# HaileyMai/Self-supervised-scene-generation-with-semantic-segmentation

Measured on NVIDIA B200. Metric: raycast fwd+bwd rays/s, higher is better.
Workload: dtype f32

## Files before the change

include/spsg_raycast.h:

```cpp
#ifndef SPSG_RAYCAST_H_
#define SPSG_RAYCAST_H_

#include <stddef.h>
#include <stdint.h>

#ifdef __cplusplus
extern "C" {
#endif

#if defined(__GNUC__)
#define SPSG_API __attribute__((visibility("default")))
#else
#define SPSG_API
#endif

#define SPSG_SEMANTIC_CHANNELS 14
#define SPSG_GRAD_CHANNELS 21

enum {
    SPSG_OK = 0,
    SPSG_ERR_INVALID_ARGUMENT = 1,
    SPSG_ERR_CUDA = 2,
    SPSG_ERR_WORKSPACE_TOO_SMALL = 3
};

enum {
    SPSG_FLAG_NO_CLIP = 1u << 0,
    SPSG_FLAG_NO_BRICK_SKIP = 1u << 1,
    SPSG_FLAG_RECORD_HITS = 1u << 2,
    SPSG_FLAG_GRADS_CLEARED = 1u << 3,
    SPSG_FLAG_SMEM_MAPS = 1u << 5,
    SPSG_FLAG_GLOBAL_MAPS = 1u << 6,
    SPSG_FLAG_PACKED_LOCS = 1u << 8,
    SPSG_FLAG_INDEX_PREBUILT = 1u << 7,
    SPSG_FLAG_DETERMINISTIC_GRADS = 1u << 4,
    SPSG_FLAG_VIEW_NORMALS = 1u << 9
};

typedef struct spsg_raycast_params {
    int32_t width, height;
    float depth_min, depth_max, thresh_sample_dist, ray_increment;
    int32_t dimx, dimy, dimz;
    int32_t num_chunks;
    int32_t views_per_chunk;
    int32_t max_pixels_per_voxel;
    int64_t num_locs;
    uint32_t flags;
    uint32_t reserved;
} spsg_raycast_params;

typedef struct spsg_loss_targets {
    const float *target_depth;
    const float *target_color;
    const float *weight_color;
    const uint8_t *target_label;
    const float *class_weight;
    float voxelsize;
    float weight_depth, weight_color_loss, weight_semantic;
} spsg_loss_targets;

typedef struct spsg_grad_buffers {
    float *d_color;
    float *d_depth;
    float *d_normal;
    float *d_semantic;
} spsg_grad_buffers;

#define SPSG_LOSS_OUT_FLOATS 8

SPSG_API const char *spsg_version(void);
SPSG_API const char *spsg_last_error(void);

SPSG_API void spsg_timing_enable(int on);
SPSG_API int spsg_timing_read(int which, double *total_ms, int *launches);

SPSG_API size_t spsg_workspace_bytes(const spsg_raycast_params *p);

SPSG_API int spsg_build_index(const int64_t *locs, int64_t num_locs, int32_t *sparse_mapping, int32_t num_chunks,
                              int32_t dimz, int32_t dimy, int32_t dimx, void *stream);

SPSG_API int spsg_raycast_forward(const spsg_raycast_params *p, const int32_t *sparse_mapping, const int64_t *locs,
                                  const float *vals_sdf, const float *vals_color, const float *vals_normal,
                                  const float *vals_semantic, const float *view_matrix, const float *intrinsics,
                                  float *image_color, float *image_depth, float *image_normal,
                                  float *image_semantic, int32_t *mapping3dto2d, int32_t *mapping3dto2d_num,
                                  void *workspace, size_t workspace_bytes, void *stream);

SPSG_API int spsg_raycast_forward_indexed(const spsg_raycast_params *p, int32_t *sparse_mapping, const int64_t *locs,
// ... 148 lines not shown
```

self-supervised-scene-generation-with-semantic-segmentation_b200/_native.py:

```python
import ctypes
import os

_HERE = os.path.dirname(os.path.abspath(__file__))
LIB_PATH = os.environ.get("SPSG_RAYCAST_LIB", os.path.join(_HERE, "lib", "libspsg_raycast.so"))

SPSG_FLAG_NO_CLIP = 1 << 0
SPSG_FLAG_NO_BRICK_SKIP = 1 << 1
SPSG_FLAG_RECORD_HITS = 1 << 2
SPSG_FLAG_GRADS_CLEARED = 1 << 3
SPSG_FLAG_DETERMINISTIC_GRADS = 1 << 4
SPSG_FLAG_SMEM_MAPS = 1 << 5
SPSG_FLAG_GLOBAL_MAPS = 1 << 6
SPSG_FLAG_INDEX_PREBUILT = 1 << 7
SPSG_FLAG_PACKED_LOCS = 1 << 8
SPSG_FLAG_VIEW_NORMALS = 1 << 9
SPSG_LOSS_OUT_FLOATS = 8
SPSG_DTYPE_F32 = 0
SPSG_DTYPE_BF16 = 1
SPSG_DEPTH_MAX_FILL_ROUNDS = 64

EXPORTS = (
    "spsg_version", "spsg_last_error", "spsg_workspace_bytes", "spsg_build_index", "spsg_raycast_forward",
    "spsg_raycast_forward_indexed", "spsg_raycast_backward", "spsg_raycast_occ", "spsg_raycast_forward_loss",
    "spsg_raycast_backward_loss", "spsg_raycast_backward_loss_upstream", "spsg_timing_enable", "spsg_timing_read",
    "spsg_normals_forward", "spsg_normals_backward", "spsg_normals_forward_views", "spsg_normals_backward_views",
    "spsg_losses2d_forward", "spsg_losses2d_backward",
    "spsg_depth_bilateral_filter", "spsg_depth_median_fill", "spsg_depth_to_cameraspace", "spsg_depth_to_normals",
    "spsg_depth_compute_normals",
    "spsg_sparsify_scratch_bytes", "spsg_sparsify_count", "spsg_sparsify_locs", "spsg_sparsify_locs_indexed",
    "spsg_dense_gather", "spsg_dense_scatter",
    "spsg_sparsify_count_bf16", "spsg_sparsify_locs_bf16", "spsg_sparsify_locs_indexed_bf16",
    "spsg_dense_gather_strided", "spsg_dense_scatter_strided",
    "spsg_labels_from_render", "spsg_pack_locs_host",
)


class Params(ctypes.Structure):
    _fields_ = [
        ("width", ctypes.c_int32), ("height", ctypes.c_int32),
        ("depth_min", ctypes.c_float), ("depth_max", ctypes.c_float),
        ("thresh_sample_dist", ctypes.c_float), ("ray_increment", ctypes.c_float),
        ("dimx", ctypes.c_int32), ("dimy", ctypes.c_int32), ("dimz", ctypes.c_int32),
        ("num_chunks", ctypes.c_int32), ("views_per_chunk", ctypes.c_int32),
        ("max_pixels_per_voxel", ctypes.c_int32),
        ("num_locs", ctypes.c_int64),
        ("flags", ctypes.c_uint32), ("reserved", ctypes.c_uint32),
    ]


class LossTargets(ctypes.Structure):
    _fields_ = [
        ("target_depth", ctypes.c_void_p), ("target_color", ctypes.c_void_p), ("weight_color", ctypes.c_void_p),
        ("target_label", ctypes.c_void_p), ("class_weight", ctypes.c_void_p),
        ("voxelsize", ctypes.c_float), ("weight_depth", ctypes.c_float), ("weight_color_loss", ctypes.c_float),
        ("weight_semantic", ctypes.c_float),
    ]


class DensePayload(ctypes.Structure):
    _fields_ = [("dense", ctypes.c_void_p), ("sparse", ctypes.c_void_p), ("channels", ctypes.c_int32),
                ("reserved", ctypes.c_int32)]


class DenseHead(ctypes.Structure):
    _fields_ = [("dense", ctypes.c_void_p), ("sparse", ctypes.c_void_p), ("strides", ctypes.c_int64 * 5),
                ("extent", ctypes.c_int64), ("channels", ctypes.c_int32), ("dtype", ctypes.c_int32)]


# ... 148 lines not shown
```

self-supervised-scene-generation-with-semantic-segmentation_b200/csrc/spsg_common.cuh:

```cuda
#pragma once

constexpr int kFineLog2 = 2;
constexpr int kFine = 1 << kFineLog2;
constexpr int kSuper = 8;
constexpr float kBoxEps = 1.0f / 64.0f;
constexpr float kFracGuard = 1.0f / 256.0f;
constexpr int kMaxFastDim = 8192;
constexpr int kLossSlots = 64;

enum { kKindSurface = 0, kKindEmpty = 1, kKindPos = 2, kKindNeg = 3 };

thread_local char g_err[512] = "";

int fail(int code, const char *msg) {
    snprintf(g_err, sizeof(g_err), "%s", msg);
    return code;
}
int fail_cuda(cudaError_t e, const char *where) {
    snprintf(g_err, sizeof(g_err), "%s: %s", where, cudaGetErrorString(e));
    return SPSG_ERR_CUDA;
}
#define CUDA_TRY(x)                                      \
    do {                                                 \
        cudaError_t e_ = (x);                            \
        if (e_ != cudaSuccess) return fail_cuda(e_, #x); \
    } while (0)

inline size_t align_up(size_t v, size_t a) { return (v + a - 1) / a * a; }

struct EventPair { cudaEvent_t a, b; };
bool g_timing = false;
std::vector<EventPair> g_ev[2];
std::mutex g_timing_mu;

struct ScopedKernelTimer {
    int which; cudaStream_t st; EventPair ev; bool on;
    ScopedKernelTimer(int w, cudaStream_t s) : which(w), st(s), on(g_timing) {
        if (on) {
            on = cudaEventCreate(&ev.a) == cudaSuccess && cudaEventCreate(&ev.b) == cudaSuccess;
            if (on) cudaEventRecord(ev.a, st);
        }
    }
    ~ScopedKernelTimer() {
        if (on) {
            cudaEventRecord(ev.b, st);
            std::lock_guard<std::mutex> lk(g_timing_mu);
            g_ev[which].push_back(ev);
        }
    }
};

struct Layout {
    int nbx, nby, nbz;
    size_t bpc;
    size_t dense_off, dense_bytes;
    int wpr;
    size_t vpc;
    size_t vbit_off, vbit_bytes;
    size_t bmap_off, bmap_bytes;
    size_t marks_off, marks_bytes;
    size_t zero_off, zero_bytes;
    size_t head_off;
    size_t tiles_off, tiles_bytes;
    size_t arrive_off, arrive_bytes;
    size_t loss_off, loss_bytes;
    size_t list_off, list_bytes;
    size_t hits_off, hits_bytes;
    size_t total;
};

Layout make_layout(const spsg_raycast_params *p) {
    Layout L;
    L.nbx = (p->dimx + kFine - 1) >> kFineLog2;
    L.nby = (p->dimy + kFine - 1) >> kFineLog2;
    L.nbz = (p->dimz + kFine - 1) >> kFineLog2;
    L.bpc = align_up((size_t)L.nbx * L.nby * L.nbz, 16);
    const int F = p->views_per_chunk > 0 ? p->views_per_chunk : 1;
    const size_t cells = (size_t)p->num_chunks * p->dimz * p->dimy * p->dimx;
    size_t off = 0;
    L.dense_off = off;
    L.dense_bytes = align_up(cells * sizeof(float), 256);
    off += L.dense_bytes;
    L.wpr = (p->dimx + 31) / 32;
    L.vpc = align_up((size_t)p->dimz * p->dimy * L.wpr, 2);
    L.vbit_off = off;
    L.vbit_bytes = align_up((size_t)p->num_chunks * L.vpc * sizeof(uint2), 256);
    off += L.vbit_bytes;
    L.bmap_off = off;
    L.bmap_bytes = align_up((size_t)p->num_chunks * L.bpc, 256);
    off += L.bmap_bytes;
    L.marks_off = off;
    L.marks_bytes = align_up((size_t)p->num_chunks * L.bpc, 256);
    off += L.marks_bytes;
    L.zero_off = off;
    L.head_off = off;
    off += 256;
    L.tiles_off = off;
    L.tiles_bytes = align_up((size_t)p->num_chunks * sizeof(int32_t), 256);
    off += L.tiles_bytes;
    L.arrive_off = off;
    L.arrive_bytes = align_up((size_t)p->num_chunks * ((L.nbz + 7) / 8) * ((L.nby + 7) / 8) * L.wpr * sizeof(int32_t), 256);
    off += L.arrive_bytes;
    L.loss_off = off;
    L.loss_bytes = align_up((size_t)kLossSlots * 8 * sizeof(double), 256);
    off += L.loss_bytes;
    L.zero_bytes = off - L.zero_off;
    L.list_off = off;
    L.list_bytes = align_up((size_t)(p->num_locs > 0 ? p->num_locs : 0) * F * 2 * sizeof(int32_t), 256);
    off += L.list_bytes;
    L.hits_off = off;
    L.hits_bytes = align_up((size_t)p->num_chunks * F * p->width * p->height * sizeof(int32_t), 256);
    off += L.hits_bytes;
    L.total = off;
    return L;
}
```

self-supervised-scene-generation-with-semantic-segmentation_b200/csrc/spsg_forward.cuh:

```cuda
#pragma once


#ifdef SPSG_STATS
__device__ unsigned long long g_stats[48];
__device__ int g_tile_stats[131072][8];
#define STAT_MAX(k, v) atomicMax(&g_stats[k], (unsigned long long)(v))
#define STAT_ADD(k, v) atomicAdd(&g_stats[k], (unsigned long long)(v))
#if SPSG_STATS == 1
#define EVT_ADD(k, v) STAT_ADD(k, v)
#else
#define EVT_ADD(k, v)
#endif
#else
#define STAT_ADD(k, v)
#define STAT_MAX(k, v)
#define EVT_ADD(k, v)
#endif

struct LossArgs {
    const float *target_depth, *target_color, *weight_color;
    const uint8_t *target_label;
    const float *class_weight;
    float voxelsize;
    double *accum;
    float *loss_out;
    int32_t *done;
    float w_depth, w_color, w_sem;
};

__device__ __forceinline__ void finalize_loss_warp(const double *acc, float *__restrict__ out, float w_depth, float w_color,
                                                   float w_sem, bool has_depth, bool has_color, bool has_sem, int lane);

struct ForwardArgs {
    const int32_t *sparse_mapping;
    const float *vals_sdf, *vals_color, *vals_normal, *vals_semantic;
    const float *view_matrix, *intrinsics;
    float *image_color, *image_depth, *image_normal, *image_semantic;
    int32_t *mapping3dto2d, *mapping3dto2d_num;
    const float *dense;
    const uint2 *vbits;
    const uint8_t *bmap;
    size_t vpc, bpc;
    int wpr;
    int maps_in_smem;
    int32_t *tile_counter;
    int32_t *list_count;
    int2 *list;
    int32_t *hits;
    int width, height;
    float depth_min, depth_max, thresh, inc;
    int dimx, dimy, dimz;
    int vx, vy, vz;
    int nbx, nby, nbz;
    int num_chunks, views, max_pixels;
    long long num_locs;
    unsigned flags;
    int vec_ok;
    float guard;
    LossArgs loss;
    spsg_grad_buffers clear;
    long long clear_rows;
};

constexpr int kTileW = 16, kTileH = 8;
constexpr int kTilePix = kTileW * kTileH;

constexpr int kWarpW = 8, kWarpH = 4;
constexpr int kFwdWarps = 24;
#ifndef SPSG_FWD_WARPS_LARGE
#define SPSG_FWD_WARPS_LARGE 28
#endif
constexpr int kFwdWarpsLarge = SPSG_FWD_WARPS_LARGE;
constexpr int kFwdThreads = kFwdWarps * 32;
constexpr int kStageFloats = 14 * 32;
__host__ __device__ constexpr size_t fwd_smem_fixed(int warps) { return 128 + (size_t)warps * kStageFloats * sizeof(float); }
constexpr size_t kFwdSmemFixed = fwd_smem_fixed(kFwdWarpsLarge);
constexpr size_t kFwdSmemMax = 232448 - 1024;

__device__ __forceinline__ float warp_sum(float v) {
#pragma unroll
    for (int o = 16; o > 0; o >>= 1) v += __shfl_xor_sync(0xffffffffu, v, o);
    return v;
}

__device__ __forceinline__ uint32_t smem_u32(const void *p) { return (uint32_t)__cvta_generic_to_shared(p); }
__device__ __forceinline__ void mbar_init(uint64_t *bar, unsigned count) {
    asm volatile("mbarrier.init.shared::cta.b64 [%0], %1;" ::"r"(smem_u32(bar)), "r"(count) : "memory");
    asm volatile("fence.mbarrier_init.release.cluster;" ::: "memory");
}
__device__ __forceinline__ void mbar_expect_tx(uint64_t *bar, unsigned bytes) {
    asm volatile("mbarrier.arrive.expect_tx.shared::cta.b64 _, [%0], %1;" ::"r"(smem_u32(bar)), "r"(bytes) : "memory");
}
__device__ __forceinline__ void bulk_copy_g2s(void *dst, const void *src, unsigned bytes, uint64_t *bar) {
    asm volatile("cp.async.bulk.shared::cluster.global.mbarrier::complete_tx::bytes [%0], [%1], %2, [%3];" ::"r"(
                     smem_u32(dst)),
                 "l"(src), "r"(bytes), "r"(smem_u32(bar))
                 : "memory");
}
// ... 178 lines not shown
            int img, view, wx0, wy0;
#ifdef SPSG_STATS
            long long clk0;
#endif
        };
        auto prepare = [&](int tile, TileRay &q) {
            const int view = tile / tiles_per_image, tt = tile - view * tiles_per_image;
            const int blk = tt >> 2, sub = tt & 3;
            const int by = blk / blocks_x, bx = blk - by * blocks_x;
            const int wx0 = (bx * 2 + (sub & 1)) * kWarpW, wy0 = (by * 2 + (sub >> 1)) * kWarpH;
            const int img = chunk * a.views + view;
            q.view = view; q.img = img; q.wx0 = wx0; q.wy0 = wy0;
            q.inside = wx0 < a.width && wy0 < a.height;
            if (q.inside) {
                const unsigned ux = wx0 + (lane & 7), uy = wy0 + (lane >> 3);
                const bool active = ux < (unsigned)a.width && uy < (unsigned)a.height;
                const unsigned pix = uy * a.width + ux;
                const size_t gpix = (size_t)img * a.width * a.height + pix;

#ifdef SPSG_STATS
                q.clk0 = clock64();
#endif
                const Ray r = setup_ray(a.view_matrix + (size_t)img * 16, a.intrinsics + (size_t)img * 4,
                                        active ? ux : 0u, active ? uy : 0u, a.depth_min, a.depth_max);
                const float invx = r.dx != 0.0f ? rcp_approx(r.dx) : 0.0f, invy = r.dy != 0.0f ? rcp_approx(r.dy) : 0.0f,
                            invz = r.dz != 0.0f ? rcp_approx(r.dz) : 0.0f;
                const float kx = r.dx != 0.0f ? ((r.dx > 0.0f ? -kBoxEps : kBoxEps) - r.camx) * invx : kInf;
                const float ky = r.dy != 0.0f ? ((r.dy > 0.0f ? -kBoxEps : kBoxEps) - r.camy) * invy : kInf;
                const float kz = r.dz != 0.0f ? ((r.dz > 0.0f ? -kBoxEps : kBoxEps) - r.camz) * invz : kInf;
                const int sxm = r.dx > 0.0f ? -1 : 0, sym = r.dy > 0.0f ? -1 : 0, szm = r.dz > 0.0f ? -1 : 0;
                float ray = r.t0, t_end = active ? r.t1 : -kInf;
                int jump_cap = 1 << 22;
                {
                    const float top = fmaxf(fabsf(r.t1), 1.0f);
                    const float ulp = __uint_as_float(__float_as_uint(top) & 0x7f800000u) * 1.1920928955078125e-07f;
                    const float cap = (0.5f * kBoxEps) / ulp;
                    jump_cap = cap < 4194304.0f ? max(1, __float2int_rd(cap)) : (1 << 22);
                }
                if (clip && active) {
                    float tin = -kInf, tout = kInf;
#define SPSG_SLAB(o, d, inv, lo, hi)                                        \
    if ((d) != 0.0f) {                                                      \
        const float ta_ = ((lo) - (o)) * (inv), tb_ = ((hi) - (o)) * (inv); \
        tin = fmaxf(tin, fminf(ta_, tb_));                                  \
        tout = fminf(tout, fmaxf(ta_, tb_));                                \
    } else if ((o) < (lo) || (o) > (hi)) {                                  \
        tin = kInf;                                                         \
        tout = -kInf;                                                       \
    }
                    SPSG_SLAB(r.camx, r.dx, invx, -kBoxEps, (float)(a.dimx - 1) + kBoxEps)
                    SPSG_SLAB(r.camy, r.dy, invy, -kBoxEps, (float)(a.dimy - 1) + kBoxEps)
                    SPSG_SLAB(r.camz, r.dz, invz, -kBoxEps, (float)(a.dimz - 1) + kBoxEps)
#undef SPSG_SLAB
                    const float margin = 0.0625f;
                    if (!(tin <= tout)) {
                        t_end = -kInf;
                    } else {
                        t_end = fminf(t_end, tout + margin);
                        while (ray < tin - margin - a.inc && ray < t_end) {
                            const int want = max(1, min(__float2int_rd((tin - margin - ray) * inv_inc) - 1, jump_cap));
                            ray = step_advance(s_steps, a.inc, ray, want);
                        }
                        for (int k = 0; k < 6 && ray < t_end; k++) {
                            const int ix = __float2int_rd(__fmaf_rn(r.dx, ray, r.camx)), iy = __float2int_rd(__fmaf_rn(r.dy, ray, r.camy)),
                                      iz = __float2int_rd(__fmaf_rn(r.dz, ray, r.camz));
                            if ((unsigned)ix < (unsigned)a.vx && (unsigned)iy < (unsigned)a.vy && (unsigned)iz < (unsigned)a.vz) break;
                            if (!skip_ok) break;
                            ray = __fadd_rn(ray, a.inc);
                        }
                    }
                }
                q.r = r; q.invx = invx; q.invy = invy; q.invz = invz; q.kx = kx; q.ky = ky; q.kz = kz;
                q.sxm = sxm; q.sym = sym; q.szm = szm; q.ray = ray; q.t_end = t_end; q.jump_cap = jump_cap;
                q.pix = pix; q.gpix = gpix; q.active = active;
            }
        };
        TileRay q;
        q.inside = false;
        if (tile < tile_limit) prepare(bind_chunk(tile), q);
        if (kSmemMaps) mbar_wait(mbar, phase);

        while (tile < tile_limit) {
            int next = tile_limit;
            if (lane == 0 && static_tiles < tile_limit) next = static_tiles + atomicAdd(counter, 1);
            if (q.inside) {
                const Ray r = q.r;
                const float invx = q.invx, invy = q.invy, invz = q.invz, kx = q.kx, ky = q.ky, kz = q.kz;
                const int sxm = q.sxm, sym = q.sym, szm = q.szm, jump_cap = q.jump_cap;
                float ray = q.ray;
                const float t_end = q.t_end;
                const unsigned pix = q.pix;
                const size_t gpix = q.gpix;
                const bool active = q.active;
                const int img = q.img, view = q.view, wx0 = q.wx0, wy0 = q.wy0;
                int hit = -1;
                float depth = 0.0f;
#ifdef SPSG_STATS
                const long long clk0 = q.clk0;
                long long clk_march = 0, clk_refine = 0;
                int my_iters = 0;
                const long long clk1 = clock64(), clk1b = clk1;
#endif

                float last_sdf = 0.0f, last_alpha = 0.0f;
                bool last_lazy = false;
                float dist = 0.0f;
// ... 327 lines not shown
```

self-supervised-scene-generation-with-semantic-segmentation_b200/csrc/spsg_prep.cuh:

```cuda
#pragma once


constexpr int kFillRegions = 3;
struct FillArgs {
    uint32_t *ptr[kFillRegions];
    size_t words[kFillRegions];
    uint32_t value[kFillRegions];
};

__global__ void __launch_bounds__(256) fill_kernel(const FillArgs a) {
    const size_t tid = (size_t)blockIdx.x * blockDim.x + threadIdx.x, stride = (size_t)gridDim.x * blockDim.x;
#pragma unroll
    for (int r = 0; r < kFillRegions; r++) {
        uint32_t *p = a.ptr[r];
        const size_t n = a.words[r];
        if (!p || n == 0) continue;
        const uint32_t v = a.value[r];
        if ((reinterpret_cast<uintptr_t>(p) & 15u) == 0) {
            const size_t n4 = n >> 2;
            uint4 *p4 = reinterpret_cast<uint4 *>(p);
            for (size_t i = tid; i < n4; i += stride) p4[i] = make_uint4(v, v, v, v);
            for (size_t i = (n4 << 2) + tid; i < n; i += stride) p[i] = v;
        } else {
            for (size_t i = tid; i < n; i += stride) p[i] = v;
        }
    }
}

__global__ void __launch_bounds__(256) index_packed_kernel(const uint32_t *__restrict__ cells, long long n,
                                                           int32_t *__restrict__ sparse_mapping,
                                                           const float *__restrict__ vals_sdf, float *__restrict__ dense,
                                                           int32_t *__restrict__ num, int views, unsigned long long grid_cells) {
    const long long i = (long long)blockIdx.x * blockDim.x + threadIdx.x;
    if (i >= n) return;
    if (num)
        for (int f = 0; f < views; f++) num[(long long)f * n + i] = 0;
    const unsigned cell = __ldg(cells + i);
    if ((unsigned long long)cell >= grid_cells) return;
    sparse_mapping[cell] = (int32_t)i;
    if (dense) dense[cell] = __ldg(vals_sdf + i);
}

template <bool kWriteIndex>
__global__ void __launch_bounds__(256) index_kernel(const longlong4 *__restrict__ locs, long long n,
                                                    int32_t *__restrict__ sparse_mapping,
                                                    const float *__restrict__ vals_sdf, float *__restrict__ dense,
                                                    int32_t *__restrict__ num, int views, int dimz, int dimy,
                                                    int dimx, int num_chunks) {
    const long long i = (long long)blockIdx.x * blockDim.x + threadIdx.x;
    if (i >= n) return;
    if (num)
        for (int f = 0; f < views; f++) num[(long long)f * n + i] = 0;
    const longlong4 l = locs[i];
    const long long z = l.x, y = l.y, x = l.z, b = l.w;
    if ((unsigned long long)z >= (unsigned long long)dimz || (unsigned long long)y >= (unsigned long long)dimy ||
        (unsigned long long)x >= (unsigned long long)dimx || b < 0 || b >= num_chunks)
        return;
    const long long cell = ((b * dimz + z) * dimy + y) * dimx + x;
    if (kWriteIndex) sparse_mapping[cell] = (int32_t)i;
    if (dense) dense[cell] = __ldg(vals_sdf + i);
}

__host__ __device__ constexpr uint8_t block_map_byte(int r1, int r2, int r3, int r4) {
    const int r[5] = {0, r1, r2, r3, r4};
    int lu = 0, le = 0;
    for (int l = 1; l <= 4; l++) {
        if (!(r[l] & 4) && (r[l] & 3) != 3) lu = l;
        if (r[l] == 0) le = l;
    }
    if (lu == 0) return 0;
    const int kind = (le == lu) ? kKindEmpty : (r[lu] & 1) ? kKindPos : kKindNeg;
    return (uint8_t)((kind << 3) | lu);
}

struct BlockLut { uint8_t v[4096]; };
constexpr BlockLut make_block_lut() {
    BlockLut t{};
    for (int i = 0; i < 4096; i++) t.v[i] = block_map_byte(i & 7, (i >> 3) & 7, (i >> 6) & 7, (i >> 9) & 7);
    return t;
}
__device__ const BlockLut kBlockLut = make_block_lut();

constexpr float kTiny = 1e-30f, kHuge = 3e38f;

__global__ void __launch_bounds__(128) cell_class_kernel(const float *__restrict__ dense, uint2 *__restrict__ vbits,
                                                         size_t vpc, uint8_t *__restrict__ marks,
                                                         int dimz, int dimy, int dimx, int wpr, int nby, int nbx,
                                                         size_t bpc, uint8_t *__restrict__ bmap, int32_t *__restrict__ arrive,
                                                         int nbz) {
    const unsigned kFull = 0xffffffffu;
    const int lane = threadIdx.x & 31;
    const int w = blockIdx.x * 4 + (threadIdx.x >> 5);
    if (w >= nby * wpr) return;
    const int yb = w / wpr, xw = w - yb * wpr;
    const int zb = blockIdx.y, chunk = blockIdx.z;
    const int y0 = yb * kFine, z0 = zb * kFine;
    const unsigned plane = (unsigned)dimy * (unsigned)dimx;
    const unsigned x = (unsigned)(xw * 32 + lane);
    const bool in_x = x < (unsigned)dimx, in_x1 = x + 1u < (unsigned)dimx;
    const unsigned o00 = ((unsigned)chunk * (unsigned)dimz + (unsigned)z0) * plane + (unsigned)y0 * (unsigned)dimx + x;
    unsigned pres[5][5], posm[5][5], negm[5][5];
#pragma unroll
    for (int dz = 0; dz < 5; dz++)
#pragma unroll
        for (int dy = 0; dy < 5; dy++) {
            const bool row = y0 + dy < dimy && z0 + dz < dimz;
            const float *__restrict__ q = dense + (o00 + (unsigned)dz * plane + (unsigned)dy * (unsigned)dimx);
            const float a = (row && in_x) ? __ldg(q) : CUDART_NAN_F;
            const float n = (row && in_x1) ? __ldg(q + 1) : CUDART_NAN_F;
            pres[dz][dy] = __ballot_sync(kFull, a == a && n == n);
            posm[dz][dy] = __ballot_sync(kFull, a > kTiny && a < kHuge && n > kTiny && n < kHuge);
            negm[dz][dy] = __ballot_sync(kFull, a < -kTiny && a > -kHuge && n < -kTiny && n > -kHuge);
        }
    unsigned any_pos = 0u, any_neg = 0u, any_mix = 0u;
    const unsigned v00 = (unsigned)chunk * (unsigned)vpc + ((unsigned)z0 * (unsigned)dimy + (unsigned)y0) * (unsigned)wpr + (unsigned)xw;
#pragma unroll
    for (int dz = 0; dz < 4; dz++)
#pragma unroll
        for (int dy = 0; dy < 4; dy++) {
            const int y = y0 + dy, z = z0 + dz;
            const unsigned v = pres[dz][dy] & pres[dz][dy + 1] & pres[dz + 1][dy] & pres[dz + 1][dy + 1];
            const unsigned vp = posm[dz][dy] & posm[dz][dy + 1] & posm[dz + 1][dy] & posm[dz + 1][dy + 1];
            const unsigned vn = negm[dz][dy] & negm[dz][dy + 1] & negm[dz + 1][dy] & negm[dz + 1][dy + 1];
            any_pos |= vp; any_neg |= vn; any_mix |= v & ~vp & ~vn;
            if (lane == 0 && y < dimy && z < dimz)
                vbits[v00 + ((unsigned)dz * (unsigned)dimy + (unsigned)dy) * (unsigned)wpr] = make_uint2(v & ~vn, v & ~vp);
        }
    if (lane < 8) {
        const int bx = xw * 8 + lane;
        if (bx < nbx)
            marks[(size_t)chunk * bpc + ((size_t)zb * nby + yb) * nbx + bx] =
                (uint8_t)((((any_pos >> (4 * lane)) & 0xfu) ? 1 : 0) | (((any_neg >> (4 * lane)) & 0xfu) ? 2 : 0) |
                          (((any_mix >> (4 * lane)) & 0xfu) ? 4 : 0));
    }
    const int sby = (nby + 7) >> 3, sbz = (nbz + 7) >> 3;
    const int sy = yb >> 3, sz = zb >> 3;
    const int rows_y = min(8, nby - sy * 8), rows_z = min(8, nbz - sz * 8);
    __threadfence();
    int prev = 0;
    if (lane == 0) prev = atomicAdd(arrive + ((size_t)chunk * sbz + sz) * sby * wpr + (size_t)sy * wpr + xw, 1);
    prev = __shfl_sync(kFull, prev, 0);
    if (prev != rows_y * rows_z - 1) return;
    __threadfence();
    const int zl = lane >> 2, yl = (lane & 3) * 2;
    uint32_t rb[2][2] = {{0u, 0u}, {0u, 0u}};
    const int nx = min(8, nbx - xw * 8);
#pragma unroll
    for (int r = 0; r < 2; r++) {
        const int gy = sy * 8 + yl + r, gz = sz * 8 + zl;
        if (gy < nby && gz < nbz) {
            const uint8_t *src = marks + (size_t)chunk * bpc + ((size_t)gz * nby + gy) * nbx + xw * 8;
            if ((nbx & 7) == 0) {
                const uint2 v2 = __ldcg(reinterpret_cast<const uint2 *>(src));
                rb[r][0] = v2.x; rb[r][1] = v2.y;
            } else {
                for (int k = 0; k < nx; k++) rb[r][k >> 2] |= (uint32_t)__ldcg(src + k) << (8 * (k & 3));
            }
        }
    }
    auto xpair = [](uint32_t v) { const uint32_t t = v | ((v >> 8) & 0x00ff00ffu); return (t & 0x00ff00ffu) | ((t & 0x00ff00ffu) << 8); };
    uint32_t r8[2];
#pragma unroll
    for (int h = 0; h < 2; h++) {
        uint32_t v = xpair(rb[0][h] | rb[1][h]);
        v |= __shfl_xor_sync(kFull, v, 4);
        r8[h] = v;
    }
    uint32_t r16[2];
#pragma unroll
    for (int h = 0; h < 2; h++) {
        uint32_t v = r8[h];
        v |= v >> 16; v |= v >> 8; v &= 0xffu;
        v |= __shfl_xor_sync(kFull, v, 1);
        v |= __shfl_xor_sync(kFull, v, 8);
        r16[h] = v;
    }
    uint32_t r32 = r16[0] | r16[1];
    r32 |= __shfl_xor_sync(kFull, r32, 2);
    r32 |= __shfl_xor_sync(kFull, r32, 16);
    const uint8_t *__restrict__ lut = kBlockLut.v;
#pragma unroll
    for (int r = 0; r < 2; r++) {
        const int gy = sy * 8 + yl + r, gz = sz * 8 + zl;
        if (gy < nby && gz < nbz) {
            uint8_t *dst = bmap + (size_t)chunk * bpc + ((size_t)gz * nby + gy) * nbx + xw * 8;
            uint32_t out[2] = {0u, 0u};
// ... 15 lines not shown
```

self-supervised-scene-generation-with-semantic-segmentation_b200/csrc/spsg_raycast.cu:

```cuda
#include <cuda_runtime.h>
#include <math_constants.h>
#include <stdint.h>
#include <stdio.h>
#include <string.h>

#include <algorithm>
#include <mutex>
#include <vector>

#include "spsg_raycast.h"

namespace {

#include "spsg_common.cuh"
#include "spsg_fp32.cuh"
#include "spsg_prep.cuh"
#include "spsg_forward.cuh"
#include "spsg_backward.cuh"
#include "spsg_losses2d.cuh"
#include "spsg_occ.cuh"
#include "spsg_normals.cuh"


int check_params(const spsg_raycast_params *p) {
// ... 23 lines not shown
        cudaDeviceGetAttribute(&sms, cudaDevAttrMultiProcessorCount, dev);
        cached[dev] = sms > 0 ? sms : 148;
    }
    return cached[dev];
}

LossArgs make_loss_args(const spsg_loss_targets *t, double *accum) {
    LossArgs L;
    memset(&L, 0, sizeof(L));
    if (t) {
        L.target_depth = t->target_depth; L.target_color = t->target_color; L.weight_color = t->weight_color;
        L.target_label = t->target_label; L.class_weight = t->class_weight; L.voxelsize = t->voxelsize;
    }
    L.accum = accum;
    L.loss_out = nullptr; L.done = nullptr;
    if (t) { L.w_depth = t->weight_depth; L.w_color = t->weight_color_loss; L.w_sem = t->weight_semantic; }
    return L;
}

int launch_forward(const spsg_raycast_params *p, bool build_index, int32_t *sparse_mapping, const int64_t *locs,
                   const float *vals_sdf, const float *vals_color, const float *vals_normal,
                   const float *vals_semantic, const float *view_matrix, const float *intrinsics, float *image_color,
                   float *image_depth, float *image_normal, float *image_semantic, int32_t *mapping3dto2d,
                   int32_t *mapping3dto2d_num, const spsg_loss_targets *targets, float *loss_out,
                   const spsg_grad_buffers *clear_grads, void *workspace, size_t workspace_bytes, cudaStream_t st) {
    if (int rc = check_params(p)) return rc;
    if (p->max_pixels_per_voxel <= 0) return fail(SPSG_ERR_INVALID_ARGUMENT, "max_pixels_per_voxel must be positive");
    if (!sparse_mapping || !view_matrix || !intrinsics || !image_color || !image_depth || !image_normal ||
        !image_semantic || !mapping3dto2d || !mapping3dto2d_num)
        return fail(SPSG_ERR_INVALID_ARGUMENT, "NULL tensor pointer");
    if (p->num_locs > 0 && (!locs || !vals_sdf || !vals_color || !vals_normal || !vals_semantic))
        return fail(SPSG_ERR_INVALID_ARGUMENT, "NULL voxel tensor pointer");
    if (!aligned16(view_matrix) || !aligned16(intrinsics))
        return fail(SPSG_ERR_INVALID_ARGUMENT, "view_matrix / intrinsics must be 16-byte aligned");
    const bool packed = (p->flags & SPSG_FLAG_PACKED_LOCS) != 0;
    if (p->num_locs > 0 && ((reinterpret_cast<uintptr_t>(vals_semantic) & 7u) || (reinterpret_cast<uintptr_t>(locs) & (packed ? 3u : 15u))))
        return fail(SPSG_ERR_INVALID_ARGUMENT, "vals_semantic must be 8-byte and locs 16-byte (packed: 4-byte) aligned");
    if (packed && !build_index) return fail(SPSG_ERR_INVALID_ARGUMENT, "packed locs need an entry point that builds the index");
    if (packed && (unsigned long long)p->num_chunks * p->dimz * p->dimy * p->dimx >= 0xffffffffull)
        return fail(SPSG_ERR_INVALID_ARGUMENT, "packed locs need fewer than 2^32 - 1 cells");
    if (reinterpret_cast<uintptr_t>(sparse_mapping) & 3u) return fail(SPSG_ERR_INVALID_ARGUMENT, "sparse_mapping must be 4-byte aligned");
    if (targets && !loss_out) return fail(SPSG_ERR_INVALID_ARGUMENT, "loss_out is NULL");
    const Layout L = make_layout(p);
    if (!workspace || workspace_bytes < L.total) return fail(SPSG_ERR_WORKSPACE_TOO_SMALL, "workspace too small");
    if (reinterpret_cast<uintptr_t>(workspace) & 255u) return fail(SPSG_ERR_INVALID_ARGUMENT, "workspace must be 256-byte aligned");
    uint8_t *ws = (uint8_t *)workspace;
    float *dense = (float *)(ws + L.dense_off);
    uint2 *vbits = (uint2 *)(ws + L.vbit_off);
    uint8_t *bmap = ws + L.bmap_off, *marks = ws + L.marks_off;
    double *accum = (double *)(ws + L.loss_off);
    const size_t cells = (size_t)p->num_chunks * p->dimz * p->dimy * p->dimx;
    const int sms = sm_count();
    const bool prebuilt = (p->flags & SPSG_FLAG_INDEX_PREBUILT) && p->num_locs > 0;

    {
        FillArgs f;
        memset(&f, 0, sizeof(f));
        f.ptr[0] = build_index ? (uint32_t *)sparse_mapping : nullptr; f.words[0] = cells; f.value[0] = 0xffffffffu;
        f.ptr[1] = (uint32_t *)dense; f.words[1] = L.dense_bytes / 4; f.value[1] = 0xffffffffu;
        if (prebuilt) {
            f.ptr[0] = (uint32_t *)mapping3dto2d_num; f.words[0] = (size_t)p->views_per_chunk * p->num_locs; f.value[0] = 0u;
            f.ptr[1] = nullptr; f.words[1] = 0;
        }
        f.ptr[2] = (uint32_t *)(ws + L.zero_off); f.words[2] = L.zero_bytes / 4; f.value[2] = 0u;
        if (clear_grads && p->num_locs > 0 &&
            (!clear_grads->d_color || !clear_grads->d_depth || !clear_grads->d_normal || !clear_grads->d_semantic))
            return fail(SPSG_ERR_INVALID_ARGUMENT, "NULL gradient pointer in clear_grads");
        const size_t vecs = ((prebuilt ? f.words[0] : cells * (build_index ? 2 : 1)) + L.zero_bytes / 4) / 4;
        const unsigned blocks = (unsigned)std::min<size_t>((vecs + 1023) / 1024 + 1, (size_t)sms * 8);
        fill_kernel<<<blocks, 256, 0, st>>>(f);
        CUDA_TRY(cudaGetLastError());
    }
    if (p->num_locs > 0 && !prebuilt) {
        const unsigned blocks = (unsigned)((p->num_locs + 255) / 256);
        if (packed)
            index_packed_kernel<<<blocks, 256, 0, st>>>((const uint32_t *)locs, p->num_locs, sparse_mapping, vals_sdf, dense,
                                                        mapping3dto2d_num, p->views_per_chunk, (unsigned long long)cells);
        else if (build_index)
            index_kernel<true><<<blocks, 256, 0, st>>>((const longlong4 *)locs, p->num_locs, sparse_mapping, vals_sdf,
                                                       dense, mapping3dto2d_num, p->views_per_chunk, p->dimz, p->dimy,
                                                       p->dimx, p->num_chunks);
        else
            index_kernel<false><<<blocks, 256, 0, st>>>((const longlong4 *)locs, p->num_locs, sparse_mapping, vals_sdf,
                                                        dense, mapping3dto2d_num, p->views_per_chunk, p->dimz, p->dimy,
                                                        p->dimx, p->num_chunks);
        CUDA_TRY(cudaGetLastError());
    }
    ForwardArgs a;
    memset(&a, 0, sizeof(a));
    const size_t map_bytes = L.vpc * sizeof(uint2) + L.bpc;
    a.maps_in_smem = kFwdSmemFixed + map_bytes <= kFwdSmemMax && !(p->flags & SPSG_FLAG_GLOBAL_MAPS) &&
                     (p->num_chunks == 1 || (p->flags & SPSG_FLAG_SMEM_MAPS));
    {
        const dim3 cgrid((unsigned)((L.nby * L.wpr + 3) / 4), (unsigned)L.nbz, (unsigned)p->num_chunks);
        cell_class_kernel<<<cgrid, 128, 0, st>>>(dense, vbits, L.vpc, marks, p->dimz, p->dimy, p->dimx, L.wpr, L.nby, L.nbx, L.bpc,
                                                 bmap, (int32_t *)(ws + L.arrive_off), L.nbz);
        CUDA_TRY(cudaGetLastError());
    }
    a.sparse_mapping = sparse_mapping;
    a.vals_sdf = vals_sdf; a.vals_color = vals_color; a.vals_normal = vals_normal; a.vals_semantic = vals_semantic;
    a.view_matrix = view_matrix; a.intrinsics = intrinsics;
    a.image_color = image_color; a.image_depth = image_depth; a.image_normal = image_normal;
    a.image_semantic = image_semantic;
    a.mapping3dto2d = mapping3dto2d; a.mapping3dto2d_num = mapping3dto2d_num;
    a.dense = dense; a.vbits = vbits; a.bmap = bmap; a.vpc = L.vpc; a.bpc = L.bpc; a.wpr = L.wpr;
    a.tile_counter = (int32_t *)(ws + L.tiles_off);
    a.num_chunks = p->num_chunks;
    a.list_count = (int32_t *)(ws + L.head_off);
    a.list = (int2 *)(ws + L.list_off);
    a.hits = (p->flags & SPSG_FLAG_RECORD_HITS) ? (int32_t *)(ws + L.hits_off) : nullptr;
    a.width = p->width; a.height = p->height;
    a.depth_min = p->depth_min; a.depth_max = p->depth_max; a.thresh = p->thresh_sample_dist; a.inc = p->ray_increment;
    a.dimx = p->dimx; a.dimy = p->dimy; a.dimz = p->dimz;
    {
        const bool maps = !(p->flags & SPSG_FLAG_NO_BRICK_SKIP) && std::max(p->dimx, std::max(p->dimy, p->dimz)) <= kMaxFastDim;
        a.vx = maps ? p->dimx - 1 : 0; a.vy = maps ? p->dimy - 1 : 0; a.vz = maps ? p->dimz - 1 : 0;
    }
    a.nbx = L.nbx; a.nby = L.nby; a.nbz = L.nbz;
    a.views = p->views_per_chunk; a.max_pixels = p->max_pixels_per_voxel;
    a.num_locs = p->num_locs;
    a.flags = p->flags;
    a.vec_ok = (p->width % 4 == 0) && aligned16(image_color) && aligned16(image_depth) && aligned16(image_normal) &&
               aligned16(image_semantic);
    {
        int k = 0;
        while ((1 << k) < std::max(p->dimx, std::max(p->dimy, p->dimz))) k++;
        a.guard = std::min(kFracGuard, std::max(ldexpf(1.0f, k - 21), ldexpf(1.0f, -18)));
    }
    a.loss = make_loss_args(targets, accum);
    a.loss.loss_out = loss_out;
    a.loss.done = (int32_t *)(ws + L.head_off) + 16;
    if (clear_grads && p->num_locs > 0) {
        a.clear = *clear_grads;
        a.clear_rows = p->num_locs;
    }
    const long long tiles_x = (p->width + kWarpW - 1) / kWarpW, tiles_y = (p->height + kWarpH - 1) / kWarpH;
    const long long all_tiles = ((tiles_x + 1) / 2) * ((tiles_y + 1) / 2) * 4 * p->views_per_chunk * p->num_chunks;
    const unsigned grid = (unsigned)std::max<long long>(1, std::min<long long>(sms, all_tiles));
    const bool large = all_tiles >= (long long)sms * 4 * kFwdWarpsLarge;
    const bool view_normals = (p->flags & SPSG_FLAG_VIEW_NORMALS) && p->views_per_chunk > 1;
    const int warps = large ? kFwdWarpsLarge : kFwdWarps;
    const size_t dyn = fwd_smem_fixed(warps) + (a.maps_in_smem ? map_bytes : 0);
    {
        static std::mutex mu;
        static bool configured[64] = {false};
        int dev = 0;
        CUDA_TRY(cudaGetDevice(&dev));
        std::lock_guard<std::mutex> lk(mu);
        if (dev < 0 || dev >= 64 || !configured[dev]) {
#define SPSG_SET_SMEM(L, M, W, VN) CUDA_TRY(cudaFuncSetAttribute(raycast_forward_kernel<L, M, W, VN>, cudaFuncAttributeMaxDynamicSharedMemorySize, (int)kFwdSmemMax))
#define SPSG_SET_SMEM_ALL(VN)                                                                                   \
    SPSG_SET_SMEM(true, true, kFwdWarps, VN); SPSG_SET_SMEM(false, true, kFwdWarps, VN);                         \
    SPSG_SET_SMEM(true, false, kFwdWarps, VN); SPSG_SET_SMEM(false, false, kFwdWarps, VN);                       \
    SPSG_SET_SMEM(true, true, kFwdWarpsLarge, VN); SPSG_SET_SMEM(false, true, kFwdWarpsLarge, VN);               \
    SPSG_SET_SMEM(true, false, kFwdWarpsLarge, VN); SPSG_SET_SMEM(false, false, kFwdWarpsLarge, VN)
            SPSG_SET_SMEM_ALL(false);
            SPSG_SET_SMEM_ALL(true);
#undef SPSG_SET_SMEM_ALL
#undef SPSG_SET_SMEM
// ... 446 lines not shown
```

Baseline: 4.888 billion.

## Splat occupied voxel bricks into per-tile depth bounds to tighten ray intervals

Adds a per-image, per-screen-tile near/far depth bound. The fill kernel computes camera matrices, and the cell classification kernel projects each non-empty brick's box onto screen tiles, recording min-near and max-far with atomics. The forward raycast intersects its box-slab interval with these tile bounds, so rays skip empty space before and after the occupied geometry and tiles with no geometry stop early. The cost is extra work, atomics and workspace during prep, and the bounds must be conservative or results change.

```diff
diff --git a/include/spsg_raycast.h b/include/spsg_raycast.h
--- a/include/spsg_raycast.h
+++ b/include/spsg_raycast.h
@@ -34,6 +34,7 @@
     SPSG_FLAG_PACKED_LOCS = 1u << 8,
     SPSG_FLAG_INDEX_PREBUILT = 1u << 7,
     SPSG_FLAG_DETERMINISTIC_GRADS = 1u << 4,
+    SPSG_FLAG_NO_TILE_BOUNDS = 1u << 10,
     SPSG_FLAG_VIEW_NORMALS = 1u << 9
 };
 
diff --git a/self-supervised-scene-generation-with-semantic-segmentation_b200/_native.py b/self-supervised-scene-generation-with-semantic-segmentation_b200/_native.py
--- a/self-supervised-scene-generation-with-semantic-segmentation_b200/_native.py
+++ b/self-supervised-scene-generation-with-semantic-segmentation_b200/_native.py
@@ -14,6 +14,7 @@
 SPSG_FLAG_INDEX_PREBUILT = 1 << 7
 SPSG_FLAG_PACKED_LOCS = 1 << 8
 SPSG_FLAG_VIEW_NORMALS = 1 << 9
+SPSG_FLAG_NO_TILE_BOUNDS = 1 << 10
 SPSG_LOSS_OUT_FLOATS = 8
 SPSG_DTYPE_F32 = 0
 SPSG_DTYPE_BF16 = 1
diff --git a/self-supervised-scene-generation-with-semantic-segmentation_b200/csrc/spsg_common.cuh b/self-supervised-scene-generation-with-semantic-segmentation_b200/csrc/spsg_common.cuh
--- a/self-supervised-scene-generation-with-semantic-segmentation_b200/csrc/spsg_common.cuh
+++ b/self-supervised-scene-generation-with-semantic-segmentation_b200/csrc/spsg_common.cuh
@@ -59,7 +59,10 @@
     size_t vbit_off, vbit_bytes;
     size_t bmap_off, bmap_bytes;
     size_t marks_off, marks_bytes;
+    size_t cams_off, cams_bytes;
+    int quads_x, quads;
     size_t zero_off, zero_bytes;
+    size_t bounds_off, bounds_bytes;
     size_t head_off;
     size_t tiles_off, tiles_bytes;
     size_t arrive_off, arrive_bytes;
@@ -92,6 +95,12 @@
     L.marks_off = off;
     L.marks_bytes = align_up((size_t)p->num_chunks * L.bpc, 256);
     off += L.marks_bytes;
+    const size_t images = (size_t)p->num_chunks * F;
+    L.cams_off = off;
+    L.cams_bytes = align_up(images * 16 * sizeof(float), 256);
+    off += L.cams_bytes;
+    L.quads_x = ((p->width + 7) / 8 + 1) / 2;
+    L.quads = L.quads_x * (((p->height + 3) / 4 + 1) / 2);
     L.zero_off = off;
     L.head_off = off;
     off += 256;
@@ -104,6 +113,9 @@
     L.loss_off = off;
     L.loss_bytes = align_up((size_t)kLossSlots * 8 * sizeof(double), 256);
     off += L.loss_bytes;
+    L.bounds_off = off;
+    L.bounds_bytes = align_up(images * L.quads * sizeof(uint2), 256);
+    off += L.bounds_bytes;
     L.zero_bytes = off - L.zero_off;
     L.list_off = off;
     L.list_bytes = align_up((size_t)(p->num_locs > 0 ? p->num_locs : 0) * F * 2 * sizeof(int32_t), 256);
diff --git a/self-supervised-scene-generation-with-semantic-segmentation_b200/csrc/spsg_forward.cuh b/self-supervised-scene-generation-with-semantic-segmentation_b200/csrc/spsg_forward.cuh
--- a/self-supervised-scene-generation-with-semantic-segmentation_b200/csrc/spsg_forward.cuh
+++ b/self-supervised-scene-generation-with-semantic-segmentation_b200/csrc/spsg_forward.cuh
@@ -44,6 +44,8 @@
     int wpr;
     int maps_in_smem;
     int32_t *tile_counter;
+    const uint2 *bounds;
+    int quads;
     int32_t *list_count;
     int2 *list;
     int32_t *hits;
@@ -328,6 +330,11 @@
                     SPSG_SLAB(r.camy, r.dy, invy, -kBoxEps, (float)(a.dimy - 1) + kBoxEps)
                     SPSG_SLAB(r.camz, r.dz, invz, -kBoxEps, (float)(a.dimz - 1) + kBoxEps)
 #undef SPSG_SLAB
+                    if (a.bounds) {
+                        const uint2 b = __ldg(a.bounds + (size_t)img * a.quads + blk);
+                        tin = fmaxf(tin, b.x ? __uint_as_float(~b.x) : kInf);
+                        tout = fminf(tout, b.x ? __uint_as_float(b.y) : -kInf);
+                    }
                     const float margin = 0.0625f;
                     if (!(tin <= tout)) {
                         t_end = -kInf;
diff --git a/self-supervised-scene-generation-with-semantic-segmentation_b200/csrc/spsg_prep.cuh b/self-supervised-scene-generation-with-semantic-segmentation_b200/csrc/spsg_prep.cuh
--- a/self-supervised-scene-generation-with-semantic-segmentation_b200/csrc/spsg_prep.cuh
+++ b/self-supervised-scene-generation-with-semantic-segmentation_b200/csrc/spsg_prep.cuh
@@ -6,10 +6,33 @@
     uint32_t *ptr[kFillRegions];
     size_t words[kFillRegions];
     uint32_t value[kFillRegions];
+    const float *view_matrix;
+    float *cams;
+    int images;
 };
+
+__device__ void camera_from_view(const float *__restrict__ M, float *__restrict__ out) {
+    double a[3][3];
+    for (int r = 0; r < 3; r++)
+        for (int c = 0; c < 3; c++) a[r][c] = M[r * 4 + c];
+    const double c00 = a[1][1] * a[2][2] - a[1][2] * a[2][1], c01 = a[1][2] * a[2][0] - a[1][0] * a[2][2],
+                 c02 = a[1][0] * a[2][1] - a[1][1] * a[2][0];
+    const double det = a[0][0] * c00 + a[0][1] * c01 + a[0][2] * c02;
+    const bool ok = det != 0.0 && isfinite(det);
+    const double inv[3][3] = {
+        {c00, a[0][2] * a[2][1] - a[0][1] * a[2][2], a[0][1] * a[1][2] - a[0][2] * a[1][1]},
+        {c01, a[0][0] * a[2][2] - a[0][2] * a[2][0], a[0][2] * a[1][0] - a[0][0] * a[1][2]},
+        {c02, a[0][1] * a[2][0] - a[0][0] * a[2][1], a[0][0] * a[1][1] - a[0][1] * a[1][0]}};
+    for (int r = 0; r < 3; r++) {
+        for (int c = 0; c < 3; c++) out[r * 4 + c] = ok ? (float)(inv[r][c] / det) : CUDART_NAN_F;
+        out[r * 4 + 3] = 0.0f;
+    }
+    out[12] = M[3]; out[13] = M[7]; out[14] = M[11]; out[15] = 0.0f;
+}
 
 __global__ void __launch_bounds__(256) fill_kernel(const FillArgs a) {
     const size_t tid = (size_t)blockIdx.x * blockDim.x + threadIdx.x, stride = (size_t)gridDim.x * blockDim.x;
+    if (a.cams && tid < (size_t)a.images) camera_from_view(a.view_matrix + tid * 16, a.cams + tid * 16);
 #pragma unroll
     for (int r = 0; r < kFillRegions; r++) {
         uint32_t *p = a.ptr[r];
@@ -83,11 +106,114 @@
 
 constexpr float kTiny = 1e-30f, kHuge = 3e38f;
 
+struct TileBoundArgs {
+    const float *cams;
+    const float *intrinsics;
+    uint2 *bounds;
+    int views, width, height, quads_x, quads;
+};
+
+struct QuadBox {
+    int qx0, qx1, qy0, qy1;
+    float near, far;
+};
+
+__device__ QuadBox project_box(const TileBoundArgs &t, int img, float x0, float x1, float y0, float y1, float z0, float z1) {
+    QuadBox out = {INT_MAX, -1, INT_MAX, -1, 0.0f, 0.0f};
+    const float4 *c4 = reinterpret_cast<const float4 *>(t.cams + (size_t)img * 16);
+    const float4 r0 = __ldg(c4), r1 = __ldg(c4 + 1), r2 = __ldg(c4 + 2), cp = __ldg(c4 + 3);
+    const float4 k = __ldg(reinterpret_cast<const float4 *>(t.intrinsics + (size_t)img * 4));
+    const float ex = fmaxf(fmaxf(x0 - cp.x, cp.x - x1), 0.0f), ey = fmaxf(fmaxf(y0 - cp.y, cp.y - y1), 0.0f),
+                ez = fmaxf(fmaxf(z0 - cp.z, cp.z - z1), 0.0f);
+    const float fx_ = fmaxf(fabsf(x0 - cp.x), fabsf(x1 - cp.x)), fy_ = fmaxf(fabsf(y0 - cp.y), fabsf(y1 - cp.y)),
+                fz_ = fmaxf(fabsf(z0 - cp.z), fabsf(z1 - cp.z));
+    float near = fmaxf(sqrtf(ex * ex + ey * ey + ez * ez) * (1.0f - 1.0f / 65536.0f) - 0.0625f, 0.0f);
+    float far = sqrtf(fx_ * fx_ + fy_ * fy_ + fz_ * fz_) * (1.0f + 1.0f / 65536.0f) + 0.0625f;
+    float umin = CUDART_INF_F, umax = -CUDART_INF_F, vmin = CUDART_INF_F, vmax = -CUDART_INF_F;
+    int front = 0, behind = 0;
+#pragma unroll
+    for (int i = 0; i < 8; i++) {
+        const float dx = (i & 1 ? x1 : x0) - cp.x, dy = (i & 2 ? y1 : y0) - cp.y, dz = (i & 4 ? z1 : z0) - cp.z;
+        const float cx = r0.x * dx + r0.y * dy + r0.z * dz, cy = r1.x * dx + r1.y * dy + r1.z * dz,
+                    cz = r2.x * dx + r2.y * dy + r2.z * dz;
+        const float sx = fabsf(r0.x * dx) + fabsf(r0.y * dy) + fabsf(r0.z * dz);
+        const float sy = fabsf(r1.x * dx) + fabsf(r1.y * dy) + fabsf(r1.z * dz);
+        const float sz = fabsf(r2.x * dx) + fabsf(r2.y * dy) + fabsf(r2.z * dz);
+        const float eps = 1e-4f * sz + 1e-6f;
+        if (cz > eps) {
+            front++;
+            const float iz = 1.0f / cz, xn = cx * iz, yn = cy * iz;
+            const float mu = fabsf(k.x) * 1e-6f * (sx + fabsf(xn) * sz) * iz + 1.0f;
+            const float mv = fabsf(k.y) * 1e-6f * (sy + fabsf(yn) * sz) * iz + 1.0f;
+            const float u = k.x * xn + k.z, v = k.y * yn + k.w;
+            umin = fminf(umin, u - mu); umax = fmaxf(umax, u + mu);
+            vmin = fminf(vmin, v - mv); vmax = fmaxf(vmax, v + mv);
+        } else if (cz < -eps) {
+            behind++;
+        }
+    }
+    if (behind == 8) return out;
+    int qx0 = 0, qx1 = t.quads_x - 1, qy0 = 0, qy1 = t.quads / t.quads_x - 1;
+    const bool finite = isfinite(near) && isfinite(far) && isfinite(umin) && isfinite(umax) && isfinite(vmin) &&
+                        isfinite(vmax);
+    if (!finite) {
+        near = 0.0f; far = CUDART_INF_F;
+    } else if (front == 8) {
+        const float lu = ceilf(fmaxf(umin, 0.0f)), hu = floorf(fminf(umax, (float)(t.width - 1)));
+        const float lv = ceilf(fmaxf(vmin, 0.0f)), hv = floorf(fminf(vmax, (float)(t.height - 1)));
+        if (!(lu <= hu && lv <= hv)) return out;
+        qx0 = (int)lu >> 4; qx1 = (int)hu >> 4; qy0 = (int)lv >> 3; qy1 = (int)hv >> 3;
+    }
+    out.qx0 = qx0; out.qx1 = qx1; out.qy0 = qy0; out.qy1 = qy1; out.near = near; out.far = far;
+    return out;
+}
+
+__device__ void splat_blocks(const TileBoundArgs &t, int chunk, unsigned nonempty, float x0, float x1, float y0, float y1,
+                             float z0, float z1, int lane) {
+    const unsigned kFull = 0xffffffffu;
+    const int k = lane & 7;
+    for (int f0 = 0; f0 < t.views; f0 += 4) {
+        const int f = f0 + (lane >> 3);
+        QuadBox q = {INT_MAX, -1, INT_MAX, -1, 0.0f, 0.0f};
+        if (((nonempty >> k) & 1u) && f < t.views) q = project_box(t, chunk * t.views + f, x0, x1, y0, y1, z0, z1);
+        int ux0 = q.qx0, ux1 = q.qx1, uy0 = q.qy0, uy1 = q.qy1;
+#pragma unroll
+        for (int o = 1; o < 8; o <<= 1) {
+            ux0 = min(ux0, __shfl_xor_sync(kFull, ux0, o)); ux1 = max(ux1, __shfl_xor_sync(kFull, ux1, o));
+            uy0 = min(uy0, __shfl_xor_sync(kFull, uy0, o)); uy1 = max(uy1, __shfl_xor_sync(kFull, uy1, o));
+        }
+        for (int g = 0; g < 4 && f0 + g < t.views; g++) {
+            const int gx0 = __shfl_sync(kFull, ux0, 8 * g), gx1 = __shfl_sync(kFull, ux1, 8 * g);
+            const int gy0 = __shfl_sync(kFull, uy0, 8 * g), gy1 = __shfl_sync(kFull, uy1, 8 * g);
+            if (gx0 > gx1 || gy0 > gy1) continue;
+            uint2 *b = t.bounds + (size_t)(chunk * t.views + f0 + g) * t.quads;
+            const int w = gx1 - gx0 + 1, n = w * (gy1 - gy0 + 1);
+            for (int base = 0; base < n; base += 32) {
+                const int i = base + lane, qy = gy0 + i / w, qx = gx0 + i % w;
+                float near = CUDART_INF_F, far = -CUDART_INF_F;
+#pragma unroll
+                for (int j = 0; j < 8; j++) {
+                    const int src = 8 * g + j;
+                    const int bx0 = __shfl_sync(kFull, q.qx0, src), bx1 = __shfl_sync(kFull, q.qx1, src);
+                    const int by0 = __shfl_sync(kFull, q.qy0, src), by1 = __shfl_sync(kFull, q.qy1, src);
+                    const float bn = __shfl_sync(kFull, q.near, src), bf = __shfl_sync(kFull, q.far, src);
+                    if (qx >= bx0 && qx <= bx1 && qy >= by0 && qy <= by1) { near = fminf(near, bn); far = fmaxf(far, bf); }
+                }
+                if (i < n && near != CUDART_INF_F) {
+                    uint2 *e = b + qy * t.quads_x + qx;
+                    atomicMax(&e->x, ~__float_as_uint(near));
+                    atomicMax(&e->y, __float_as_uint(far));
+                }
+            }
+        }
+    }
+}
+
 __global__ void __launch_bounds__(128) cell_class_kernel(const float *__restrict__ dense, uint2 *__restrict__ vbits,
                                                          size_t vpc, uint8_t *__restrict__ marks,
                                                          int dimz, int dimy, int dimx, int wpr, int nby, int nbx,
                                                          size_t bpc, uint8_t *__restrict__ bmap, int32_t *__restrict__ arrive,
-                                                         int nbz) {
+                                                         int nbz, const TileBoundArgs tb) {
     const unsigned kFull = 0xffffffffu;
     const int lane = threadIdx.x & 31;
     const int w = blockIdx.x * 4 + (threadIdx.x >> 5);
@@ -100,6 +226,7 @@
     const bool in_x = x < (unsigned)dimx, in_x1 = x + 1u < (unsigned)dimx;
     const unsigned o00 = ((unsigned)chunk * (unsigned)dimz + (unsigned)z0) * plane + (unsigned)y0 * (unsigned)dimx + x;
     unsigned pres[5][5], posm[5][5], negm[5][5];
+    bool any_voxel = false;
 #pragma unroll
     for (int dz = 0; dz < 5; dz++)
 #pragma unroll
@@ -108,6 +235,7 @@
             const float *__restrict__ q = dense + (o00 + (unsigned)dz * plane + (unsigned)dy * (unsigned)dimx);
             const float a = (row && in_x) ? __ldg(q) : CUDART_NAN_F;
             const float n = (row && in_x1) ? __ldg(q + 1) : CUDART_NAN_F;
+            if (dz < 4 && dy < 4) any_voxel |= a == a;
             pres[dz][dy] = __ballot_sync(kFull, a == a && n == n);
             posm[dz][dy] = __ballot_sync(kFull, a > kTiny && a < kHuge && n > kTiny && n < kHuge);
             negm[dz][dy] = __ballot_sync(kFull, a < -kTiny && a > -kHuge && n < -kTiny && n > -kHuge);
@@ -126,12 +254,21 @@
             if (lane == 0 && y < dimy && z < dimz)
                 vbits[v00 + ((unsigned)dz * (unsigned)dimy + (unsigned)dy) * (unsigned)wpr] = make_uint2(v & ~vn, v & ~vp);
         }
+    const unsigned any_vox = __ballot_sync(kFull, any_voxel);
     if (lane < 8) {
         const int bx = xw * 8 + lane;
         if (bx < nbx)
             marks[(size_t)chunk * bpc + ((size_t)zb * nby + yb) * nbx + bx] =
                 (uint8_t)((((any_pos >> (4 * lane)) & 0xfu) ? 1 : 0) | (((any_neg >> (4 * lane)) & 0xfu) ? 2 : 0) |
-                          (((any_mix >> (4 * lane)) & 0xfu) ? 4 : 0));
+                          (((any_mix >> (4 * lane)) & 0xfu) ? 4 : 0) | (((any_vox >> (4 * lane)) & 0xfu) ? 8 : 0));
+    }
+    if (tb.bounds && any_vox) {
+        const int k = lane & 7, bx = xw * 8 + k;
+        const float x0 = (float)(bx * kFine), x1 = fminf((float)(bx * kFine + kFine), (float)(dimx - 1));
+        const float y1 = fminf((float)(y0 + kFine), (float)(dimy - 1)), z1 = fminf((float)(z0 + kFine), (float)(dimz - 1));
+        const unsigned nonempty = __ballot_sync(kFull, lane < 8 && bx < nbx && ((any_vox >> (4 * k)) & 0xfu) && x0 < x1 &&
+                                                           (float)y0 < y1 && (float)z0 < z1);
+        if (nonempty) splat_blocks(tb, chunk, nonempty, x0, x1, (float)y0, y1, (float)z0, z1, lane);
     }
     const int sby = (nby + 7) >> 3, sbz = (nbz + 7) >> 3;
     const int sy = yb >> 3, sz = zb >> 3;
diff --git a/self-supervised-scene-generation-with-semantic-segmentation_b200/csrc/spsg_raycast.cu b/self-supervised-scene-generation-with-semantic-segmentation_b200/csrc/spsg_raycast.cu
--- a/self-supervised-scene-generation-with-semantic-segmentation_b200/csrc/spsg_raycast.cu
+++ b/self-supervised-scene-generation-with-semantic-segmentation_b200/csrc/spsg_raycast.cu
@@ -99,6 +99,14 @@
     const size_t cells = (size_t)p->num_chunks * p->dimz * p->dimy * p->dimx;
     const int sms = sm_count();
     const bool prebuilt = (p->flags & SPSG_FLAG_INDEX_PREBUILT) && p->num_locs > 0;
+    const long long tiles_all = (((p->width + kWarpW - 1) / kWarpW + 1) / 2) * (((p->height + kWarpH - 1) / kWarpH + 1) / 2) * 4ll *
+                                p->views_per_chunk * p->num_chunks;
+    const bool tile_bounds = tiles_all > (long long)sms * kFwdWarps &&
+                             !(p->flags & (SPSG_FLAG_NO_CLIP | SPSG_FLAG_NO_BRICK_SKIP | SPSG_FLAG_NO_TILE_BOUNDS)) &&
+                             std::max(p->dimx, std::max(p->dimy, p->dimz)) <= kMaxFastDim && p->depth_min >= 0.0f &&
+                             p->depth_max > p->depth_min && p->depth_max < 3.0e38f;
+    float *cams = (float *)(ws + L.cams_off);
+    uint2 *bounds = (uint2 *)(ws + L.bounds_off);
 
     {
         FillArgs f;
@@ -110,11 +118,13 @@
             f.ptr[1] = nullptr; f.words[1] = 0;
         }
         f.ptr[2] = (uint32_t *)(ws + L.zero_off); f.words[2] = L.zero_bytes / 4; f.value[2] = 0u;
+        if (tile_bounds) { f.view_matrix = view_matrix; f.cams = cams; f.images = p->num_chunks * p->views_per_chunk; }
         if (clear_grads && p->num_locs > 0 &&
             (!clear_grads->d_color || !clear_grads->d_depth || !clear_grads->d_normal || !clear_grads->d_semantic))
             return fail(SPSG_ERR_INVALID_ARGUMENT, "NULL gradient pointer in clear_grads");
         const size_t vecs = ((prebuilt ? f.words[0] : cells * (build_index ? 2 : 1)) + L.zero_bytes / 4) / 4;
-        const unsigned blocks = (unsigned)std::min<size_t>((vecs + 1023) / 1024 + 1, (size_t)sms * 8);
+        const unsigned blocks = (unsigned)std::max<size_t>(std::min<size_t>((vecs + 1023) / 1024 + 1, (size_t)sms * 8),
+                                                           ((size_t)f.images + 255) / 256);
         fill_kernel<<<blocks, 256, 0, st>>>(f);
         CUDA_TRY(cudaGetLastError());
     }
@@ -139,9 +149,12 @@
     a.maps_in_smem = kFwdSmemFixed + map_bytes <= kFwdSmemMax && !(p->flags & SPSG_FLAG_GLOBAL_MAPS) &&
                      (p->num_chunks == 1 || (p->flags & SPSG_FLAG_SMEM_MAPS));
     {
+        TileBoundArgs tb;
+        tb.cams = cams; tb.intrinsics = intrinsics; tb.bounds = tile_bounds ? bounds : nullptr;
+        tb.views = p->views_per_chunk; tb.width = p->width; tb.height = p->height; tb.quads_x = L.quads_x; tb.quads = L.quads;
         const dim3 cgrid((unsigned)((L.nby * L.wpr + 3) / 4), (unsigned)L.nbz, (unsigned)p->num_chunks);
         cell_class_kernel<<<cgrid, 128, 0, st>>>(dense, vbits, L.vpc, marks, p->dimz, p->dimy, p->dimx, L.wpr, L.nby, L.nbx, L.bpc,
-                                                 bmap, (int32_t *)(ws + L.arrive_off), L.nbz);
+                                                 bmap, (int32_t *)(ws + L.arrive_off), L.nbz, tb);
         CUDA_TRY(cudaGetLastError());
     }
     a.sparse_mapping = sparse_mapping;
@@ -152,6 +165,8 @@
     a.mapping3dto2d = mapping3dto2d; a.mapping3dto2d_num = mapping3dto2d_num;
     a.dense = dense; a.vbits = vbits; a.bmap = bmap; a.vpc = L.vpc; a.bpc = L.bpc; a.wpr = L.wpr;
     a.tile_counter = (int32_t *)(ws + L.tiles_off);
+    a.bounds = tile_bounds ? bounds : nullptr;
+    a.quads = L.quads;
     a.num_chunks = p->num_chunks;
     a.list_count = (int32_t *)(ws + L.head_off);
     a.list = (int2 *)(ws + L.list_off);
```

Measured after the change: 5.017 billion (median of 6 runs). 2.6% higher.
